# izhengfan/se2lam

Hardware: AMD Instinct MI355X
Metric: BA GN-iters/s (200 KF, 20k pts) (higher is better)
Workload: dtype f64; 1 GPU; globalBA-window 200 KF / 20000 landmarks / 119817 EdgeSE2XYZ + 199 PreEdgeSE2, LM optimize(10) (config 4 formulation, SURVEY D3); parallelism=single GPU

## Files before the change

se2lam_amd/csrc/ba.hip:

```cpp
#include <algorithm>
#include <atomic>
#include <chrono>
#include <cmath>
#include <cstdlib>
#include <functional>
#include <limits>
#include <mutex>
#include <thread>
#include <tuple>
#include <memory>
#include <unordered_map>

#include "common.h"
#include "se3_math.h"
#include "ba_device.h"
#include "ba_window.h"

using namespace se2gpu;
using namespace se2gpu::badev;

namespace {



// ... 154 lines not shown
        }
    }
}
template <bool FUSED>
__global__ __launch_bounds__(kBlock) void k_linearize(CamDev cam, int L, const int* __restrict__ lm_ptr,
                                                       const int* __restrict__ e_kf, const double* __restrict__ e_uv,
                                                       const double* __restrict__ e_info,
                                                       const double* __restrict__ poses,
                                                       const uint8_t* __restrict__ fixed,
                                                       const double* __restrict__ lms, double* W,
                                                       double* Hpp_e, double* bp_e,
                                                       double* __restrict__ Hll, double* __restrict__ bl, double lambda,
                                                       double* __restrict__ Ainv, double* __restrict__ zeta,
                                                       double* __restrict__ Dg,
                                                       const BaCtl* __restrict__ ctl, const double* __restrict__ poses_b,
                                                       const double* __restrict__ lms_b) {
    d_linearize<FUSED>(blockIdx.x, cam, L, lm_ptr, e_kf, e_uv, e_info, poses, fixed, lms, W, Hpp_e, bp_e, Hll, bl, lambda, Ainv, zeta, Dg, ctl, poses_b, lms_b);
}


__device__ __forceinline__ void d_odometry(const unsigned bx, int O, const int* __restrict__ o_i, const int* __restrict__ o_j,
                           const double* __restrict__ o_meas, const double* __restrict__ o_info,
                           const double* __restrict__ poses, const uint8_t* __restrict__ fixed,
                           double* __restrict__ Oii, double* __restrict__ Ojj, double* __restrict__ Oij,
                           double* __restrict__ obi, double* __restrict__ obj, const BaCtl* __restrict__ ctl,
                           const double* __restrict__ poses_b) {
    if (ctl && ctl->sel) poses = poses_b;
    const int k = bx * blockDim.x + threadIdx.x;
    if (k >= O) return;
    const int i = o_i[k], j = o_j[k];
    double e[3], A[9], B[9];
// ... 195 lines not shown
    const int i = o_i[k], j = o_j[k];
    pre_se2(poses + 3 * i, poses + 3 * j, o_meas + 3 * k, e, A, B);
    const double* W = o_info + 9 * k;
    for (int r = 0; r < 3; ++r) {
        omr[r] = -(W[r * 3] * e[0] + W[r * 3 + 1] * e[1] + W[r * 3 + 2] * e[2]);
        for (int c = 0; c < 3; ++c) {
            WA[r * 3 + c] = W[r * 3] * A[c] + W[r * 3 + 1] * A[3 + c] + W[r * 3 + 2] * A[6 + c];
            WB[r * 3 + c] = W[r * 3] * B[c] + W[r * 3 + 1] * B[3 + c] + W[r * 3 + 2] * B[6 + c];
        }
    }
}

constexpr int kGrpPerWG = 28;
constexpr int kChunk = 16;

__device__ __forceinline__ void d_reduce2(const unsigned bx, int P, int ld, int nwg_off, double lambda, int root,
                                                     const int4* __restrict__ grp, const int* __restrict__ blk_a,
                                                     const int* __restrict__ blk_b, const int* __restrict__ pair_i,
                                                     const int* __restrict__ pair_j, const int* __restrict__ blk_odo,
                                                     const double* __restrict__ W,
                                                     const double* __restrict__ Dg,
                                                     const uint8_t* __restrict__ fixed, const int* __restrict__ pose_ptr,
                                                     const int* __restrict__ pose_edges, const int* __restrict__ podo_ptr,
                                                     const int* __restrict__ podo_item, const int* __restrict__ o_i,
                                                     const int* __restrict__ o_j, const double* __restrict__ o_meas,
                                                     const double* __restrict__ o_info, const double* __restrict__ poses,
                                                     double* __restrict__ S, double* __restrict__ bp,
                                                     const BaCtl* __restrict__ ctl, const double* __restrict__ poses_b,
                                                     unsigned* __restrict__ epoch, const int* __restrict__ pose_off, int nsys) {
    const int n = pose_off ? nsys : 3 * P;
    __shared__ double part[kGrpPerWG][9];
    __shared__ double dpart[kBlock / 64][12];
    const int ndiag = (P + 1 + 7) & ~7;
    if ((int)bx >= ndiag) {
        const int bid = (int)bx - ndiag;
        const int nwg_pad = (nwg_off + 7) & ~7;
        const int wg = (bid & 7) * (nwg_pad >> 3) + (bid >> 3);
        if (wg >= nwg_off) return;
        const int lane = threadIdx.x & 63, gw = lane / 9, en = lane - 9 * gw;
        const int g = gw < 7 ? (int)(threadIdx.x >> 6) * 7 + gw : kGrpPerWG;
        int4 d = make_int4(-1, 0, 0, 0);
        if (g < kGrpPerWG) d = grp[(size_t)wg * kGrpPerWG + g];
        if (ctl) {
            if (ctl->done) return;
// ... 52 lines not shown
            for (int t = 0; t < ng; ++t) tot += part[g + t][en];
            double out = 0.0;
            if (free_ab) {
                out = -tot;
                if (od >= 0) {
                    double e[3], A[9], B[9], WA[9], WB[9], omr[3];
                    odo_terms(poses, fixed, o_i, o_j, o_meas, o_info, od >> 1, e, A, B, WA, WB, omr);
                    const int rr = (od & 1) ? c : r, cc = (od & 1) ? r : c;
                    const double a0 = rr == 0 ? A[0] : (rr == 1 ? A[1] : A[2]), a1 = rr == 0 ? A[3] : (rr == 1 ? A[4] : A[5]),
                                 a2 = rr == 0 ? A[6] : (rr == 1 ? A[7] : A[8]);
                    const double b0 = cc == 0 ? WB[0] : (cc == 1 ? WB[1] : WB[2]), b1 = cc == 0 ? WB[3] : (cc == 1 ? WB[4] : WB[5]),
                                 b2 = cc == 0 ? WB[6] : (cc == 1 ? WB[7] : WB[8]);
                    out += a0 * b0 + a1 * b1 + a2 * b2;
                }
            }
            S[(size_t)(ca + r) * ld + cb + c] = out;
            S[(size_t)(cb + c) * ld + ca + r] = out;
        }
        return;
    }
    if (ctl) {
        if (ctl->done) return;
        if (ctl->sel) poses = poses_b;
        lambda = ctl->lambda;
    }
    const int p = (int)bx;
    if (p > P) return;
    const int lane = threadIdx.x & 63, wv = threadIdx.x >> 6;
    double* __restrict__ bs = S + (size_t)n * ld;
    if (p == P) {
        for (size_t t = (size_t)n * ld + n + threadIdx.x; t < (size_t)ld * ld; t += kBlock) S[t] = 0.0;
        if (threadIdx.x == 0) {
            S[(size_t)ld * ld + 2] = 0.0;
            *epoch += 1u;
        }
        return;
    }
    double acc[12] = {0, 0, 0, 0, 0, 0, 0, 0, 0, 0, 0, 0};
    const bool fa = fixed[p];
    __shared__ double odoc[8][12];
    const int no = fa ? 0 : podo_ptr[p + 1] - podo_ptr[p];
    if ((int)threadIdx.x >= kBlock - 8 && (int)threadIdx.x - (kBlock - 8) < min(no, 8)) {
        const int t = podo_ptr[p] + (int)threadIdx.x - (kBlock - 8);
        const int k = podo_item[t] >> 1, isj = podo_item[t] & 1;
        double e[3], A[9], B[9], WA[9], WB[9], omr[3];
        odo_terms(poses, fixed, o_i, o_j, o_meas, o_info, k, e, A, B, WA, WB, omr);
        double J[9], WJ[9];
// ... 54 lines not shown
#pragma unroll
            for (int q = 0; q < 3; ++q) {
                const double j0 = isj ? B[3 * q] : A[3 * q], j1 = isj ? B[3 * q + 1] : A[3 * q + 1], j2 = isj ? B[3 * q + 2] : A[3 * q + 2];
                const double w0 = isj ? WB[3 * q] : WA[3 * q], w1 = isj ? WB[3 * q + 1] : WA[3 * q + 1], w2 = isj ? WB[3 * q + 2] : WA[3 * q + 2];
                jr[q] = r == 0 ? j0 : (r == 1 ? j1 : j2);
                wc[q] = i < 9 ? (c == 0 ? w0 : (c == 1 ? w1 : w2)) : omr[q];
            }
            v += jr[0] * wc[0] + jr[1] * wc[1] + jr[2] * wc[2];
        }
        if (i < 9) {
            const int r = i / 3, c = i - 3 * r;
            double out;
            if (fa) out = (r == c && root) ? 1.0 : 0.0;
            else out = v + ((r == c && root) ? lambda : 0.0);
            const int cp = pose_off ? pose_off[p] : 3 * p;
            S[(size_t)(cp + r) * ld + cp + c] = out;
        } else {
            const int r = i - 9;
            const double gz = dpart[0][9 + r] + dpart[1][9 + r] + dpart[2][9 + r] + dpart[3][9 + r];
            bs[(pose_off ? pose_off[p] : 3 * p) + r] = fa ? 0.0 : v - gz;
            bp[(size_t)p * 3 + r] = fa ? 0.0 : v;
        }
    }
}
__global__ __launch_bounds__(kBlock) void k_reduce2(int P, int ld, int nwg_off, double lambda, int root,
                                                     const int4* __restrict__ grp, const int* __restrict__ blk_a,
                                                     const int* __restrict__ blk_b, const int* __restrict__ pair_i,
                                                     const int* __restrict__ pair_j, const int* __restrict__ blk_odo,
                                                     const double* __restrict__ W,
                                                     const double* __restrict__ Dg,
                                                     const uint8_t* __restrict__ fixed, const int* __restrict__ pose_ptr,
                                                     const int* __restrict__ pose_edges, const int* __restrict__ podo_ptr,
                                                     const int* __restrict__ podo_item, const int* __restrict__ o_i,
                                                     const int* __restrict__ o_j, const double* __restrict__ o_meas,
                                                     const double* __restrict__ o_info, const double* __restrict__ poses,
                                                     double* __restrict__ S, double* __restrict__ bp,
                                                     const BaCtl* __restrict__ ctl, const double* __restrict__ poses_b,
                                                     unsigned* __restrict__ epoch, const int* __restrict__ pose_off, int nsys) {
// ... 212 lines not shown
        if (wall_clock64() - t0 > 200000000ll) return false;
    }
    return true;
}

constexpr int kVfyRecords = 64, kVfyChk = 8 + 8 * kVfyRecords;
__device__ inline unsigned long long wave_xor64(unsigned long long v) {
#pragma unroll
    for (int m = 1; m < 64; m <<= 1) v ^= (unsigned long long)__shfl_xor((long long)v, m);
    return v;
}
__device__ inline unsigned long long bits4(d2_t a, d2_t b) {
    return (unsigned long long)__double_as_longlong(a.x) ^ (unsigned long long)__double_as_longlong(a.y) ^
           (unsigned long long)__double_as_longlong(b.x) ^ (unsigned long long)__double_as_longlong(b.y);
}
template <bool VERIFY>
__device__ __forceinline__ void d_chol_tiles(const unsigned bx_dispatch, const double* __restrict__ A, double* __restrict__ PUB,
                                                     double* __restrict__ YU, int ld, int n,
                                                     int nbc, const int4* __restrict__ tasks, const int* __restrict__ deps,
                                                     const int* __restrict__ col_src,
                                                     unsigned* __restrict__ flagA, unsigned* __restrict__ flagR,
                                                     const unsigned* __restrict__ epoch_ptr, double* __restrict__ fail,
                                                     long long* __restrict__ dbg, const BaCtl* __restrict__ ctl,
                                                     double* __restrict__ xout, unsigned long long* __restrict__ vfy,
                                                     unsigned long long* __restrict__ head, int ntask) {
    if (ctl && ctl->done) return;
    __shared__ unsigned task_s;
    if (head) {
        if (threadIdx.x == 0) {
            const unsigned c = __hip_atomic_fetch_add(reinterpret_cast<unsigned*>(head), 1u, __ATOMIC_RELAXED, __HIP_MEMORY_SCOPE_AGENT);
            if (c == (unsigned)ntask - 1u) __hip_atomic_store(reinterpret_cast<unsigned*>(head), 0u, __ATOMIC_RELAXED, __HIP_MEMORY_SCOPE_AGENT);
// ... 61 lines not shown
        acc += __shfl_xor(acc, 4);
        if ((tid & 7) == 0 && kNB * r + row < n) {
            const int dst = col_src ? col_src[kNB * r + row] : kNB * r + row;
            if (dst >= 0) xout[dst] = acc;
        }
        return;
    }
    const bool isR = (tk.x >> 16) != 0;
    const int i = tk.x & 0xffff, j = tk.y;
    const bool isDiag = !isR && i == j;
    const int wv = tid >> 6, ln = tid & 63;
    const int qi = 16 * (wv >> 1), qj = 16 * (wv & 1);
    const int orow = qi + (ln >> 4), ocol = qj + (ln & 15);
    const int arow = ln & 15, acol = ln >> 4;
    d4_t T0 = {0, 0, 0, 0}, D0, accT = {0, 0, 0, 0}, accD = {0, 0, 0, 0};
#pragma unroll
    for (int v = 0; v < 4; ++v) {
        D0[v] = A[(size_t)(kNB * j + orow + 4 * v) * ld + kNB * j + ocol];
        if (!isR && !isDiag) T0[v] = A[(size_t)(kNB * i + orow + 4 * v) * ld + kNB * j + ocol];
    }
    const int sr = ln >> 1, sc = 8 * wv + 4 * (ln & 1);
    for (int dq = tk.z; dq < tk.w; ++dq) {
        const int dep = deps_s[dq - tk.z];
        const int m = dep & 0x7fff;
        const bool hasT = (dep >> 15) != 0;
        __syncthreads();
        if (!ok_s) {
            if (tid == 0) fail[0] = 1e6;
            return;
        }
        const bool lazy = dq + 1 < tk.w;
        const unsigned* f0 = flagA + ((size_t)j * nbc + m) * kSlabs + wv;
        const unsigned* f1 = hasT ? (isR ? flagR : flagA) + ((size_t)i * nbc + m) * kSlabs + wv : f0;
        const int need = dq - tk.z + 1;
// ... 205 lines not shown
    if (stamp && tid == 192) stamp[5] = wall_clock64();
}
template <bool VERIFY>
__global__ __launch_bounds__(256) void k_chol_tiles(const double* __restrict__ A, double* __restrict__ PUB,
                                                     double* __restrict__ YU, int ld, int n,
                                                     int nbc, const int4* __restrict__ tasks, const int* __restrict__ deps,
                                                     const int* __restrict__ col_src,
                                                     unsigned* __restrict__ flagA, unsigned* __restrict__ flagR,
                                                     const unsigned* __restrict__ epoch_ptr, double* __restrict__ fail,
                                                     long long* __restrict__ dbg, const BaCtl* __restrict__ ctl,
                                                     double* __restrict__ xout, unsigned long long* __restrict__ vfy,
                                                     unsigned long long* __restrict__ head, int ntask) {
    d_chol_tiles<VERIFY>(blockIdx.x, A, PUB, YU, ld, n, nbc, tasks, deps, col_src, flagA, flagR, epoch_ptr, fail, dbg, ctl, xout, vfy, head, ntask);
}

__global__ __launch_bounds__(256) void k_chol_apply(const double* __restrict__ A, const double* __restrict__ R, int ld,
                                                     int n, double* __restrict__ x, const BaCtl* __restrict__ ctl,
                                                     const int* __restrict__ col_src) {
    if (ctl && ctl->done) return;
    const int r = blockIdx.x * 4 + threadIdx.x / 64;
    const int lane = threadIdx.x & 63;
    if (r >= n) return;
    const double* y = A + (size_t)n * ld;
    double acc = 0.0;
    for (int c = r + lane; c < n; c += 64) acc += R[(size_t)r * ld + c] * y[c];
    acc = wave_sum(acc);
    const int dst = col_src ? col_src[r] : r;
    if (lane == 0 && dst >= 0) x[dst] = acc;
}

// ... 1353 lines not shown
    DevBuf<double> Hpl, Hpp_e, bp_e, Hll, bl, Dinv, z, Y, Dg, Hpp, bp, Oii, Ojj, Oij, obi, obj;
    DevBuf<double> red_own, xp, part, scal, diag3, Rinv;
    DevBuf<double> red_packed;
    DevBuf<int4> chol_tasks;
    DevBuf<int> chol_deps;
    DevBuf<int> pose_off;
    DevBuf<int> col_src;
    std::vector<int> h_pose_off;
    DevBuf<uint8_t> plan_nz;
    DevBuf<double> plan_nzd;
    PinBuf<uint8_t> h_plan_nz;
    DevBuf<uint8_t> solver_arena;
    int nsys = 0;
    int solve_depth = 0;
    DevBuf<unsigned> chol_flags;
    DevBuf<unsigned long long> chol_head;
    DevBuf<unsigned long long> chol_vfy;
    DevBuf<int> plan_place;
    DevBuf<unsigned> fin_counter;
    DevBuf<unsigned long long> l0_acc;
    int chol_ntask = 0;
    struct GraphSlot { int iters = -1, mode = -1; hipGraphExec_t exec = nullptr; unsigned long stamp = 0; };
    static constexpr int kGraphSlots = 3;
    GraphSlot graphs[kGraphSlots];
    unsigned long graph_clock = 0;
    void drop_graphs() {
        for (auto& g : graphs) {
            if (g.exec) (void)hipGraphExecDestroy(g.exec);
            g = GraphSlot{};
        }
// ... 725 lines not shown
        if (sw_best != w) ring(w, sw_best, 0);
    }
}

int ba_copy_stream(int device, hipStream_t* out) {
    static std::mutex mu;
    static hipStream_t streams[64] = {};
    std::lock_guard<std::mutex> lk(mu);
    SE2_REQUIRE(device >= 0 && device < 64, SE2GPU_ERR_INVALID, "device %d", device);
    if (!streams[device]) SE2_HIP(hipStreamCreateWithFlags(&streams[device], hipStreamNonBlocking));
    *out = streams[device];
    return SE2GPU_OK;
}

int ba_allreduce(se2gpu_ba* h, double* ptr, size_t count);

int ba_upload_graph(se2gpu_ba* h) {
    static const bool trace = [] { const char* e = getenv("SE2GPU_BA_INIT_TRACE"); return e && e[0] == '1'; }();
    const auto t_begin = std::chrono::steady_clock::now();
    auto lap = [&](const char* what) {
        if (trace)
            std::fprintf(stderr, "[ba init] %-28s %8.1f us\n", what,
                         std::chrono::duration<double, std::micro>(std::chrono::steady_clock::now() - t_begin).count());
    };
    const int P = (int)h->pose_ids.size(), L = (int)h->lm_ids.size();
    const int E = h->bulk_E ? h->bulk_E : (int)h->he_kf.size(), O_in = h->model ? (int)h->odo3.size() : (int)h->odo.size();
    const int D = h->D, ps = h->ps, gpw = h->model ? kGrpPerWG3 : kGrpPerWG;
    const int DS = D * (D + 1) / 2;
    SE2_REQUIRE(P > 0, SE2GPU_ERR_STATE, "initialize: no pose vertices");
    SE2_REQUIRE(!h->model || (h->world == 1 && !h->allreduce), SE2GPU_ERR_STATE, "the SE3 model is single-GPU");
// ... 482 lines not shown
        SE2_HIP(hipMemsetAsync(h->chol_flags.p, 0, 2 * kSlabs * (size_t)nt2 * nbc2 * sizeof(unsigned), st));
        SE2_CHECK(h->chol_head.reserve(1));
        SE2_HIP(hipMemsetAsync(h->chol_head.p, 0, sizeof(unsigned long long), st));
        static const bool verify = [] { const char* e = getenv("SE2GPU_BA_CHOL_VERIFY"); return e && e[0] == '1'; }();
        if (verify) {
            const size_t words = kVfyChk + 2 * 2 * kSlabs * (size_t)nt2 * nbc2;
            SE2_CHECK(h->chol_vfy.reserve(words));
            SE2_HIP(hipMemsetAsync(h->chol_vfy.p, 0, words * sizeof(unsigned long long), st));
        } else {
            h->chol_vfy.release();
        }
        const char* env = getenv("SE2GPU_BA_CHOL");
        h->chol_steps = (env && std::strcmp(env, "steps") == 0) || nt2 > 64 || h->chol_fallback;
        const char* tr = getenv("SE2GPU_BA_CHOL_TRACE");
        if (tr && tr[0] == '1') {
            SE2_CHECK(h->chol_trace.reserve(16 * (size_t)h->chol_ntask));
            SE2_HIP(hipMemsetAsync(h->chol_trace.p, 0, 16 * (size_t)h->chol_ntask * sizeof(long long), st));
        }
        lap("solve plan");
    }
    SE2_HIP(hipStreamSynchronize(st));
    if (device_plan) {
        int nwg = 0;
        std::memcpy(&nwg, h->h_scal.p, sizeof(int));
        SE2_REQUIRE(nwg <= h->grp_cap_wg, SE2GPU_ERR_CAPACITY, "device plan: %d workgroups exceed the bound %d", nwg, h->grp_cap_wg);
        h->nwg_off = std::max(nwg, 1);
    }
    lap("synchronise");
    h->bulk_E = 0;
    h->bulk_kf = h->bulk_lm = nullptr;
    h->bulk_uv = h->bulk_info = nullptr;
    h->initialized = true;
    h->est_valid = false;
    static std::atomic<unsigned long> serial{0};
    h->init_serial = ++serial;
    drain.armed = false;
    return SE2GPU_OK;
}


inline int ba_join(se2gpu_ba* h) {
    if (h->join_event) {
// ... 18 lines not shown
    const unsigned stride = gridDim.x * 256, t0 = blockIdx.x * 256 + threadIdx.x;
    for (unsigned i = t0; i < it.np; i += stride) it.dst_p[i] = it.src_p[i];
    for (unsigned i = t0; i < it.nl; i += stride) it.dst_l[i] = it.src_l[i];
}

struct Bufs {
    const BaCtl* c;
    double *pa, *pb, *la, *lb;
};
inline Bufs bufs(se2gpu_ba* h, bool ctl) {
    if (ctl) return Bufs{h->ctl.p, h->poses_a.p, h->poses_b.p, h->lms_a.p, h->lms_b.p};
    return Bufs{nullptr, h->poses, h->poses_t, h->lms, h->lms_t};
}


int ba_linearize(se2gpu_ba* h, double fuse_lambda, bool ctl = false) {
    hipStream_t st = h->stream;
    const Bufs B = bufs(h, ctl);
    if (h->model == 2) {
        SE2_LAUNCH(h->prof, st, "k4_terms", k4_terms, grid1((size_t)h->P + h->O, 64), dim3(64), 0, h->P, h->O, B.pa, h->fixed.p,
                   h->prior_has.p, h->prior_meas.p, h->prior_info.p, h->ph.p, h->pb.p, h->slot_a.p, h->slot_ptr.p, h->pe_i.p,
                   h->pe_j.p, h->pe_meas.p, h->pe_info.p, h->Oii.p, h->Ojj.p, h->Oij.p, h->obi.p, h->obj.p, B.c, B.pb);
        SE2_HIP(hipGetLastError());
        return SE2GPU_OK;
    }
    if (h->model) {
        if (fuse_lambda >= 0.0)
            SE2_LAUNCH(h->prof, st, "k3_linearize", (k3_linearize<true>), grid1((size_t)h->L * kGroup, kBlock), dim3(kBlock), 0,
                       h->cam3, h->L, h->lm_ptr.p, h->e_kf.p, h->e_uv.p, h->e_info.p, B.pa, h->fixed.p, B.la, h->Hpl.p,
                       h->Hpp_e.p, h->bp_e.p, h->Hll.p, h->bl.p, fuse_lambda, h->Dinv.p, h->z.p, h->Y.p, h->Dg.p, B.c, B.pb, B.lb);
        else
            SE2_LAUNCH(h->prof, st, "k3_linearize", (k3_linearize<false>), grid1((size_t)h->L * kGroup, kBlock), dim3(kBlock), 0,
                       h->cam3, h->L, h->lm_ptr.p, h->e_kf.p, h->e_uv.p, h->e_info.p, B.pa, h->fixed.p, B.la, h->Hpl.p,
                       h->Hpp_e.p, h->bp_e.p, h->Hll.p, h->bl.p, 0.0, h->Dinv.p, h->z.p, h->Y.p, h->Dg.p, B.c, B.pb, B.lb);
        SE2_LAUNCH(h->prof, st, "k3_terms", k3_terms, grid1((size_t)h->P + h->O, 64), dim3(64), 0, h->P, h->O, B.pa, h->fixed.p,
                   h->prior_has.p, h->prior_meas.p, h->prior_info.p, h->pb.p, h->o_i.p, h->o_j.p, h->o_meas.p, h->o_info.p,
                   h->Oii.p, h->Ojj.p, h->Oij.p, h->obi.p, h->obj.p, B.c, B.pb);
        SE2_HIP(hipGetLastError());
        return SE2GPU_OK;
    }
    if (fuse_lambda >= 0.0)
        SE2_LAUNCH(h->prof, st, "k_linearize", (k_linearize<true>), grid1((size_t)h->L * kGroup, kBlock), dim3(kBlock), 0,
                   h->cam, h->L, h->lm_ptr.p, h->e_kf.p, h->e_uv.p, h->e_info.p, B.pa, h->fixed.p, B.la, h->Hpl.p,
                   h->Hpp_e.p, h->bp_e.p, h->Hll.p, h->bl.p, fuse_lambda, h->Dinv.p, h->z.p, h->Dg.p, B.c, B.pb, B.lb);
    else
        SE2_LAUNCH(h->prof, st, "k_linearize0", (k_linearize<false>), grid1((size_t)h->L * kGroup, kBlock), dim3(kBlock), 0,
                   h->cam, h->L, h->lm_ptr.p, h->e_kf.p, h->e_uv.p, h->e_info.p, B.pa, h->fixed.p, B.la, h->Hpl.p,
                   h->Hpp_e.p, h->bp_e.p, h->Hll.p, h->bl.p, 0.0, h->Dinv.p, h->z.p, h->Dg.p, B.c, B.pb, B.lb);
    SE2_HIP(hipGetLastError());
    return SE2GPU_OK;
}

int ba_pose_blocks(se2gpu_ba* h, const double* poses, bool ctl = false, bool odometry_only = false) {
    hipStream_t st = h->stream;
    if (h->O) {
        if (ctl)
            SE2_LAUNCH(h->prof, st, "k_odometry", k_odometry, grid1(h->O, 64), dim3(64), 0, h->O, h->o_i.p, h->o_j.p,
                       h->o_meas.p, h->o_info.p, h->poses_a.p, h->fixed.p, h->Oii.p, h->Ojj.p, h->Oij.p, h->obi.p, h->obj.p,
                       (const BaCtl*)h->ctl.p, (const double*)h->poses_b.p);
        else
            SE2_LAUNCH(h->prof, st, "k_odometry", k_odometry, grid1(h->O, 64), dim3(64), 0, h->O, h->o_i.p, h->o_j.p,
                       h->o_meas.p, h->o_info.p, poses, h->fixed.p, h->Oii.p, h->Ojj.p, h->Oij.p, h->obi.p, h->obj.p,
                       (const BaCtl*)nullptr, (const double*)nullptr);
    }
    if (!odometry_only)
        SE2_LAUNCH(h->prof, st, "k_pose_reduce", k_pose_reduce, grid1((size_t)h->P * 64, kBlock), dim3(kBlock), 0, h->P,
                   h->pose_ptr.p, h->pose_edges.p, h->Hpp_e.p, h->bp_e.p, h->podo_ptr.p, h->podo_item.p, h->Oii.p,
                   h->Ojj.p, h->obi.p, h->obj.p, h->Hpp.p, h->bp.p);
    SE2_HIP(hipGetLastError());
    return SE2GPU_OK;
}

int ba_reduce(se2gpu_ba* h, double lambda, int schur, bool ctl = false) {
    hipStream_t st = h->stream;
    double* S = h->red;
    const Bufs B = bufs(h, ctl);
    if (h->model) {
        const double* pinfo = h->model == 2 ? h->ph.p : h->prior_info.p;
        if (schur && h->model == 1)
            SE2_LAUNCH(h->prof, st, "k3_schur_lm", k3_schur_lm, grid1((size_t)h->L * kGroup, kBlock), dim3(kBlock), 0, h->L,
                       lambda, h->lm_ptr.p, h->Hll.p, h->bl.p, h->Hpl.p, h->Hpp_e.p, h->bp_e.p, h->Dinv.p, h->z.p, h->Y.p,
                       h->Dg.p, B.c, schur == 2 ? 0 : 1);
        SE2_LAUNCH(h->prof, st, "k3_reduce2", k3_reduce2, dim3(((h->P + 1 + 7) & ~7) + ((h->nwg_off + 7) & ~7)), dim3(kBlock), 0,
                   h->P, h->ld, h->nwg_off, lambda, h->grp.p, h->blk_a.p, h->blk_b.p, h->pair_i.p, h->pair_j.p, h->blk_odo.p,
                   h->Y.p, h->Hpl.p, h->Dg.p, h->fixed.p, h->pose_ptr.p, h->pose_edges.p, h->podo_ptr.p, h->podo_item.p,
                   h->prior_has.p, pinfo, h->pb.p, h->Oii.p, h->Ojj.p, h->Oij.p, h->obi.p, h->obj.p, S, h->bp.p, B.c,
                   &h->ctl.p->epoch);
        SE2_HIP(hipGetLastError());
        return SE2GPU_OK;
    }
    if (schur) SE2_CHECK(ba_linearize(h, lambda, ctl));
    SE2_LAUNCH(h->prof, st, "k_reduce2", k_reduce2, dim3(((h->P + 1 + 7) & ~7) + ((h->nwg_off + 7) & ~7)), dim3(kBlock), 0, h->P, h->ld, h->nwg_off,
               lambda, h->root, h->grp.p, h->blk_a.p, h->blk_b.p, h->pair_i.p, h->pair_j.p, h->blk_odo.p,
               h->Hpl.p, h->Dg.p, h->fixed.p, h->pose_ptr.p, h->pose_edges.p,
               h->podo_ptr.p, h->podo_item.p, h->o_i.p, h->o_j.p, h->o_meas.p, h->o_info.p, B.pa, S, h->bp.p, B.c, B.pb,
               &h->ctl.p->epoch, (const int*)h->pose_off.p, h->nsys);
    if (h->O && h->odo_fallback) {
        SE2_LAUNCH(h->prof, st, "k_odometry", k_odometry, grid1(h->O, 64), dim3(64), 0, h->O, h->o_i.p, h->o_j.p,
                   h->o_meas.p, h->o_info.p, h->poses, h->fixed.p, h->Oii.p, h->Ojj.p, h->Oij.p, h->obi.p, h->obj.p,
                   (const BaCtl*)nullptr, (const double*)nullptr);
        SE2_LAUNCH(h->prof, st, "k_reduce_odo", k_reduce_odo, grid1((size_t)h->O * 9, 256), dim3(256), 0, h->O, h->ld,
                   h->o_i.p, h->o_j.p, h->Oij.p, S);
    }
    SE2_HIP(hipGetLastError());
    return SE2GPU_OK;
}
// ... 145 lines not shown
        const int skip = (fault && !h->chol_faulted && h->chol_ntask > 1) ? 1 : 0;
        h->chol_faulted = true;
        if (h->chol_vfy.p)
            SE2_LAUNCH(h->prof, st, "k_chol_tiles", k_chol_tiles<true>, dim3(h->chol_ntask - skip), dim3(256), 0, A, Rm, YU, ld, n, nbc,
                       h->chol_tasks.p + skip, (const int*)h->chol_deps.p, (const int*)h->col_src.p, flagA, flagR, &h->ctl.p->epoch,
                       fail, h->chol_trace.p, c, h->xp.p, h->chol_vfy.p, head, h->chol_ntask - skip);
        else
            SE2_LAUNCH(h->prof, st, "k_chol_tiles", k_chol_tiles<false>, dim3(h->chol_ntask - skip), dim3(256), 0, A, Rm, YU, ld, n, nbc,
                       h->chol_tasks.p + skip, (const int*)h->chol_deps.p, (const int*)h->col_src.p, flagA, flagR, &h->ctl.p->epoch,
                       fail, h->chol_trace.p, c, h->xp.p, (unsigned long long*)nullptr, head, h->chol_ntask - skip);
    }
    SE2_HIP(hipGetLastError());
    return SE2GPU_OK;
}

int ba_lambda_init(se2gpu_ba* h) {
    hipStream_t st = h->stream;
    if (h->model) {
        SE2_LAUNCH(h->prof, st, "k3_pose_diag", k3_pose_diag, grid1((size_t)h->P * 64, kBlock), dim3(kBlock), 0, h->P,
                   h->pose_ptr.p, h->pose_edges.p, h->Hpp_e.p, h->fixed.p, h->prior_has.p,
                   h->model == 2 ? h->ph.p : h->prior_info.p, h->podo_ptr.p, h->podo_item.p, h->Oii.p, h->Ojj.p, h->diag3.p);
        SE2_LAUNCH(h->prof, st, "k_maxdiag", k_maxdiag, dim3(1), dim3(1024), 0, h->L, h->Hll.p, h->P, h->diag3.p,
                   h->fixed.p, h->scal.p, 6, 0, h->ctl.p);
        SE2_HIP(hipGetLastError());
        return SE2GPU_OK;
    }
    const bool sharded = h->allreduce && h->world > 1;
    const size_t nd = 3 * (size_t)h->P;
    if (!sharded) {
        SE2_CHECK(ba_pose_blocks(h, h->poses, true, true));
// ... 71 lines not shown
                   0.0, h->lm_ptr.p, h->e_kf.p, h->e_uv.p, h->e_info.p, B.pa, h->fixed.p, B.la,
                   step ? h->xp.p : (const double*)nullptr, h->z.p, (const double*)h->Hpl.p, h->bl.p, B.lb, h->part.p, B.c, B.pb, FinArgs{},
                   (const double*)h->Dinv.p);
        SE2_LAUNCH(h->prof, st, "k_finalize", k_finalize, dim3(1), dim3(1024), 0, h->L ? h->nparts : 0, h->part.p, h->P,
                   0.0, B.pa, h->fixed.p, h->xp.p, h->bp.p, B.pb, h->O, h->o_i.p, h->o_j.p, h->o_meas.p,
                   h->o_info.p, h->root, scal, h->d_mail, seq, h->ctl.p, step ? 1 : 0, sharded ? 0 : 1, note ? 1 : 0,
                   (const volatile int*)h->d_stop);
        if (sharded) {
            SE2_CHECK(ba_allreduce(h, scal, 4));
            hipLaunchKernelGGL(k_lm_decide, dim3(1), dim3(256), 0, st, h->ctl.p, scal, step ? 1 : 0, note ? 1 : 0,
                               h->d_mail, seq, (const volatile int*)h->d_stop);
        }
        SE2_HIP(hipGetLastError());
        return SE2GPU_OK;
    };
    if (first) {
        SE2_CHECK(evaluate(false, false));
        if (lm) {
            SE2_CHECK(ba_linearize(h, -1.0, true));
            SE2_CHECK(ba_lambda_init(h));
            SE2_CHECK(ba_reduce(h, 0.0, 3, true));
        } else {
            SE2_CHECK(ba_linearize(h, 0.0, true));
            SE2_CHECK(ba_reduce(h, 0.0, 0, true));
        }
    } else {
        if (know_retry != 1) SE2_CHECK(ba_linearize(h, 0.0, true));
        SE2_CHECK(ba_reduce(h, 0.0, !lm ? 0 : know_retry == 0 ? 0 : know_retry == 1 ? 3 : (h->model ? 2 : 0), true));
    }
    SE2_CHECK(ba_allreduce_system(h));
    SE2_CHECK(ba_solve(h, true));
    SE2_CHECK(evaluate(true, notify));
    return SE2GPU_OK;
}


template <typename... A>
struct Packed {
    int nblk;
    std::tuple<A...> args;
};
template <auto Body, int BS, typename... A>
__global__ __launch_bounds__(BS) void k_batched(const Packed<A...>* __restrict__ p) {
// ... 1613 lines not shown
```

Measured before the change: 6519 iters/s.

## Fuse Schur reduction into tiled Cholesky kernel with per-tile readiness counters

Merges the reduced-camera-system assembly (k_reduce2) into the dataflow Cholesky launch. Reduction blocks publish S entries with agent-scope stores and bump per-32x32-tile ready counters. Cholesky task blocks spin until the tiles they need are complete, using an expected-count table precomputed at setup and scaled by a generation counter bumped in linearize. This removes a kernel boundary so factorization can overlap assembly, at the cost of spin-waits, atomics on every S write, and a co-residency requirement checked through occupancy.

```diff
diff --git a/se2lam_amd/csrc/ba.hip b/se2lam_amd/csrc/ba.hip
--- a/se2lam_amd/csrc/ba.hip
+++ b/se2lam_amd/csrc/ba.hip
@@ -192,7 +192,13 @@
                                                        double* __restrict__ Ainv, double* __restrict__ zeta,
                                                        double* __restrict__ Dg,
                                                        const BaCtl* __restrict__ ctl, const double* __restrict__ poses_b,
-                                                       const double* __restrict__ lms_b) {
+                                                       const double* __restrict__ lms_b, unsigned* __restrict__ prep_epoch,
+                                                       unsigned long long* __restrict__ prep_gen, double* __restrict__ prep_fail) {
+    if (prep_gen && blockIdx.x == 0 && threadIdx.x == 0 && !(ctl && ctl->done)) {
+        *prep_epoch += 1u;
+        *prep_gen += 1ull;
+        *prep_fail = 0.0;
+    }
     d_linearize<FUSED>(blockIdx.x, cam, L, lm_ptr, e_kf, e_uv, e_info, poses, fixed, lms, W, Hpp_e, bp_e, Hll, bl, lambda, Ainv, zeta, Dg, ctl, poses_b, lms_b);
 }
 
@@ -418,7 +424,20 @@
 constexpr int kGrpPerWG = 28;
 constexpr int kChunk = 16;
 
-__device__ __forceinline__ void d_reduce2(const unsigned bx, int P, int ld, int nwg_off, double lambda, int root,
+constexpr int kSTile = 32;
+template <bool PUB>
+__device__ __forceinline__ void s_put(double* __restrict__ S, int ld, int row, int col, double v, unsigned* tl, int nt) {
+    double* p = S + (size_t)row * ld + col;
+    if constexpr (PUB) {
+        __hip_atomic_store(p, v, __ATOMIC_RELAXED, __HIP_MEMORY_SCOPE_AGENT);
+        const int ti = row / kSTile, tj = col / kSTile;
+        if (ti >= tj) atomicOr(tl + ((ti * nt + tj) >> 5), 1u << ((ti * nt + tj) & 31));
+    } else {
+        *p = v;
+    }
+}
+template <bool PUB>
+__device__ __forceinline__ void d_reduce2_body(const unsigned bx, int P, int ld, int nwg_off, double lambda, int root,
                                                      const int4* __restrict__ grp, const int* __restrict__ blk_a,
                                                      const int* __restrict__ blk_b, const int* __restrict__ pair_i,
                                                      const int* __restrict__ pair_j, const int* __restrict__ blk_odo,
@@ -431,7 +450,8 @@
                                                      const double* __restrict__ o_info, const double* __restrict__ poses,
                                                      double* __restrict__ S, double* __restrict__ bp,
                                                      const BaCtl* __restrict__ ctl, const double* __restrict__ poses_b,
-                                                     unsigned* __restrict__ epoch, const int* __restrict__ pose_off, int nsys) {
+                                                     unsigned* __restrict__ epoch, const int* __restrict__ pose_off, int nsys,
+                                                     unsigned* tl = nullptr, int nt = 0) {
     const int n = pose_off ? nsys : 3 * P;
     __shared__ double part[kGrpPerWG][9];
     __shared__ double dpart[kBlock / 64][12];
@@ -514,8 +534,8 @@
                     out += a0 * b0 + a1 * b1 + a2 * b2;
                 }
             }
-            S[(size_t)(ca + r) * ld + cb + c] = out;
-            S[(size_t)(cb + c) * ld + ca + r] = out;
+            s_put<PUB>(S, ld, ca + r, cb + c, out, tl, nt);
+            s_put<PUB>(S, ld, cb + c, ca + r, out, tl, nt);
         }
         return;
     }
@@ -527,10 +547,9 @@
     const int p = (int)bx;
     if (p > P) return;
     const int lane = threadIdx.x & 63, wv = threadIdx.x >> 6;
-    double* __restrict__ bs = S + (size_t)n * ld;
     if (p == P) {
-        for (size_t t = (size_t)n * ld + n + threadIdx.x; t < (size_t)ld * ld; t += kBlock) S[t] = 0.0;
-        if (threadIdx.x == 0) {
+        for (size_t t = (size_t)n * ld + n + threadIdx.x; t < (size_t)ld * ld; t += kBlock) s_put<PUB>(S, ld, (int)(t / ld), (int)(t % ld), 0.0, tl, nt);
+        if (threadIdx.x == 0 && epoch) {
             S[(size_t)ld * ld + 2] = 0.0;
             *epoch += 1u;
         }
@@ -615,14 +634,30 @@
             if (fa) out = (r == c && root) ? 1.0 : 0.0;
             else out = v + ((r == c && root) ? lambda : 0.0);
             const int cp = pose_off ? pose_off[p] : 3 * p;
-            S[(size_t)(cp + r) * ld + cp + c] = out;
+            s_put<PUB>(S, ld, cp + r, cp + c, out, tl, nt);
         } else {
             const int r = i - 9;
             const double gz = dpart[0][9 + r] + dpart[1][9 + r] + dpart[2][9 + r] + dpart[3][9 + r];
-            bs[(pose_off ? pose_off[p] : 3 * p) + r] = fa ? 0.0 : v - gz;
+            s_put<PUB>(S, ld, n, (pose_off ? pose_off[p] : 3 * p) + r, fa ? 0.0 : v - gz, tl, nt);
             bp[(size_t)p * 3 + r] = fa ? 0.0 : v;
         }
     }
+}
+__device__ __forceinline__ void d_reduce2(const unsigned bx, int P, int ld, int nwg_off, double lambda, int root,
+                                          const int4* __restrict__ grp, const int* __restrict__ blk_a,
+                                          const int* __restrict__ blk_b, const int* __restrict__ pair_i,
+                                          const int* __restrict__ pair_j, const int* __restrict__ blk_odo,
+                                          const double* __restrict__ W, const double* __restrict__ Dg,
+                                          const uint8_t* __restrict__ fixed, const int* __restrict__ pose_ptr,
+                                          const int* __restrict__ pose_edges, const int* __restrict__ podo_ptr,
+                                          const int* __restrict__ podo_item, const int* __restrict__ o_i,
+                                          const int* __restrict__ o_j, const double* __restrict__ o_meas,
+                                          const double* __restrict__ o_info, const double* __restrict__ poses,
+                                          double* __restrict__ S, double* __restrict__ bp,
+                                          const BaCtl* __restrict__ ctl, const double* __restrict__ poses_b,
+                                          unsigned* __restrict__ epoch, const int* __restrict__ pose_off, int nsys) {
+    d_reduce2_body<false>(bx, P, ld, nwg_off, lambda, root, grp, blk_a, blk_b, pair_i, pair_j, blk_odo, W, Dg, fixed, pose_ptr, pose_edges,
+                          podo_ptr, podo_item, o_i, o_j, o_meas, o_info, poses, S, bp, ctl, poses_b, epoch, pose_off, nsys);
 }
 __global__ __launch_bounds__(kBlock) void k_reduce2(int P, int ld, int nwg_off, double lambda, int root,
                                                      const int4* __restrict__ grp, const int* __restrict__ blk_a,
@@ -865,7 +900,7 @@
     return (unsigned long long)__double_as_longlong(a.x) ^ (unsigned long long)__double_as_longlong(a.y) ^
            (unsigned long long)__double_as_longlong(b.x) ^ (unsigned long long)__double_as_longlong(b.y);
 }
-template <bool VERIFY>
+template <bool VERIFY, bool SAGENT = false>
 __device__ __forceinline__ void d_chol_tiles(const unsigned bx_dispatch, const double* __restrict__ A, double* __restrict__ PUB,
                                                      double* __restrict__ YU, int ld, int n,
                                                      int nbc, const int4* __restrict__ tasks, const int* __restrict__ deps,
@@ -957,10 +992,26 @@
     const int orow = qi + (ln >> 4), ocol = qj + (ln & 15);
     const int arow = ln & 15, acol = ln >> 4;
     d4_t T0 = {0, 0, 0, 0}, D0, accT = {0, 0, 0, 0}, accD = {0, 0, 0, 0};
-#pragma unroll
-    for (int v = 0; v < 4; ++v) {
-        D0[v] = A[(size_t)(kNB * j + orow + 4 * v) * ld + kNB * j + ocol];
-        if (!isR && !isDiag) T0[v] = A[(size_t)(kNB * i + orow + 4 * v) * ld + kNB * j + ocol];
+    if constexpr (SAGENT) {
+        d2_t q[4], z0 = {0, 0}, z1 = {0, 0};
+#pragma unroll
+        for (int v = 0; v < 4; ++v) q[v] = load_agent(A + (size_t)(kNB * j + orow + 4 * v) * ld + kNB * j + (ocol & ~1));
+        SE2_WAIT_VM6(q[0], q[1], q[2], q[3], z0, z1);
+#pragma unroll
+        for (int v = 0; v < 4; ++v) D0[v] = (ocol & 1) ? q[v].y : q[v].x;
+        if (!isR && !isDiag) {
+#pragma unroll
+            for (int v = 0; v < 4; ++v) q[v] = load_agent(A + (size_t)(kNB * i + orow + 4 * v) * ld + kNB * j + (ocol & ~1));
+            SE2_WAIT_VM6(q[0], q[1], q[2], q[3], z0, z1);
+#pragma unroll
+            for (int v = 0; v < 4; ++v) T0[v] = (ocol & 1) ? q[v].y : q[v].x;
+        }
+    } else {
+#pragma unroll
+        for (int v = 0; v < 4; ++v) {
+            D0[v] = A[(size_t)(kNB * j + orow + 4 * v) * ld + kNB * j + ocol];
+            if (!isR && !isDiag) T0[v] = A[(size_t)(kNB * i + orow + 4 * v) * ld + kNB * j + ocol];
+        }
     }
     const int sr = ln >> 1, sc = 8 * wv + 4 * (ln & 1);
     for (int dq = tk.z; dq < tk.w; ++dq) {
@@ -1196,6 +1247,106 @@
     d_chol_tiles<VERIFY>(blockIdx.x, A, PUB, YU, ld, n, nbc, tasks, deps, col_src, flagA, flagR, epoch_ptr, fail, dbg, ctl, xout, vfy, head, ntask);
 }
 
+struct Reduce2Args {
+    int P, ld, nwg_off;
+    double lambda;
+    int root;
+    const int4* grp;
+    const int *blk_a, *blk_b, *pair_i, *pair_j, *blk_odo;
+    const double *W, *Dg;
+    const uint8_t* fixed;
+    const int *pose_ptr, *pose_edges, *podo_ptr, *podo_item, *o_i, *o_j;
+    const double *o_meas, *o_info, *poses;
+    double *S, *bp;
+    const BaCtl* ctl;
+    const double* poses_b;
+    const int* pose_off;
+    int nsys;
+};
+static_assert(kNB == kSTile, "the tile-ready counters count tiles of the dense solve");
+constexpr int kTileWords = 64 * 64 / 32;
+
+__device__ __forceinline__ void d_reduce_task(unsigned bx, const Reduce2Args& a, int nt, unsigned long long* __restrict__ ready) {
+    __shared__ unsigned tl[kTileWords];
+    for (int t = threadIdx.x; t < kTileWords; t += kBlock) tl[t] = 0u;
+    __syncthreads();
+    d_reduce2_body<true>(bx, a.P, a.ld, a.nwg_off, a.lambda, a.root, a.grp, a.blk_a, a.blk_b, a.pair_i, a.pair_j, a.blk_odo, a.W, a.Dg,
+                         a.fixed, a.pose_ptr, a.pose_edges, a.podo_ptr, a.podo_item, a.o_i, a.o_j, a.o_meas, a.o_info, a.poses, a.S, a.bp,
+                         a.ctl, a.poses_b, (unsigned*)nullptr, a.pose_off, a.nsys, tl, nt);
+    asm volatile("s_waitcnt vmcnt(0)" ::: "memory");
+    __syncthreads();
+    const int words = (nt * nt + 31) >> 5;
+    for (int w = threadIdx.x; w < words; w += kBlock) {
+        unsigned m = tl[w];
+        while (m) {
+            const int b = __builtin_ctz(m);
+            m &= m - 1u;
+            __hip_atomic_fetch_add(ready + 32 * w + b, 1ull, __ATOMIC_RELAXED, __HIP_MEMORY_SCOPE_AGENT);
+        }
+    }
+}
+__global__ __launch_bounds__(kBlock) void k_chol_fused_expect(Reduce2Args a, unsigned long long* __restrict__ expect) {
+    d_reduce_task(blockIdx.x, a, a.ld / kNB, expect);
+}
+__device__ inline bool ready_wait(const unsigned long long* c, unsigned long long want) {
+    const long long t0 = wall_clock64();
+    while (__hip_atomic_load(c, __ATOMIC_RELAXED, __HIP_MEMORY_SCOPE_AGENT) != want) {
+        __builtin_amdgcn_s_sleep(2);
+        if (wall_clock64() - t0 > 200000000ll) return false;
+    }
+    return true;
+}
+template <bool VERIFY>
+__global__ __launch_bounds__(256) void k_chol_tiles_fused(Reduce2Args ra, int nred, unsigned long long* __restrict__ ready,
+                                                          const unsigned long long* __restrict__ expect,
+                                                          const unsigned long long* __restrict__ gen_ptr,
+                                                          const double* __restrict__ A, double* __restrict__ PUB,
+                                                          double* __restrict__ YU, int ld, int n,
+                                                          int nbc, const int4* __restrict__ tasks, const int* __restrict__ deps,
+                                                          const int* __restrict__ col_src,
+                                                          unsigned* __restrict__ flagA, unsigned* __restrict__ flagR,
+                                                          const unsigned* __restrict__ epoch_ptr, double* __restrict__ fail,
+                                                          long long* __restrict__ dbg, const BaCtl* __restrict__ ctl,
+                                                          double* __restrict__ xout, unsigned long long* __restrict__ vfy,
+                                                          unsigned long long* __restrict__ head, int ntask) {
+    if (ctl && ctl->done) return;
+    const int nt = ld / kNB;
+    if ((int)blockIdx.x < nred) {
+        if (dbg && blockIdx.x == 0 && threadIdx.x == 0) dbg[16 * (size_t)ntask] = wall_clock64();
+        d_reduce_task(blockIdx.x, ra, nt, ready);
+        return;
+    }
+    __shared__ unsigned task_s;
+    __shared__ int ok_s;
+    if (threadIdx.x == 0) {
+        const unsigned c = __hip_atomic_fetch_add(reinterpret_cast<unsigned*>(head), 1u, __ATOMIC_RELAXED, __HIP_MEMORY_SCOPE_AGENT);
+        if (c == (unsigned)ntask - 1u) __hip_atomic_store(reinterpret_cast<unsigned*>(head), 0u, __ATOMIC_RELAXED, __HIP_MEMORY_SCOPE_AGENT);
+        task_s = c;
+        ok_s = 1;
+    }
+    __syncthreads();
+    const unsigned t = task_s;
+    const int4 tk = tasks[t];
+    if ((tk.x >> 16) != 2) {
+        if (threadIdx.x == 0) {
+            long long* stamp = dbg ? dbg + (size_t)t * 16 : nullptr;
+            if (stamp) stamp[8] = wall_clock64();
+            const unsigned long long g = *gen_ptr;
+            const int i = tk.x & 0xffff, j = tk.y;
+            const int td = j * nt + j, tt = ((tk.x >> 16) == 0 && i != j) ? i * nt + j : td;
+            ok_s = (ready_wait(ready + td, expect[td] * g) && ready_wait(ready + tt, expect[tt] * g)) ? 1 : 0;
+            if (stamp) stamp[9] = wall_clock64();
+        }
+        __syncthreads();
+        if (!ok_s) {
+            if (threadIdx.x == 0) fail[0] = 1e6;
+            return;
+        }
+    }
+    d_chol_tiles<VERIFY, true>(t, A, PUB, YU, ld, n, nbc, tasks, deps, col_src, flagA, flagR, epoch_ptr, fail, dbg, ctl, xout, vfy,
+                               (unsigned long long*)nullptr, ntask);
+}
+
 __global__ __launch_bounds__(256) void k_chol_apply(const double* __restrict__ A, const double* __restrict__ R, int ld,
                                                      int n, double* __restrict__ x, const BaCtl* __restrict__ ctl,
                                                      const int* __restrict__ col_src) {
@@ -2579,6 +2730,8 @@
     int nsys = 0;
     int solve_depth = 0;
     DevBuf<unsigned> chol_flags;
+    DevBuf<unsigned long long> fz;
+    bool fused = false;
     DevBuf<unsigned long long> chol_head;
     DevBuf<unsigned long long> chol_vfy;
     DevBuf<int> plan_place;
@@ -3334,6 +3487,38 @@
 }
 
 int ba_allreduce(se2gpu_ba* h, double* ptr, size_t count);
+
+Reduce2Args ba_reduce2_args(se2gpu_ba* h, const BaCtl* ctl, const double* poses, const double* poses_b) {
+    return Reduce2Args{h->P, h->ld, h->nwg_off, 0.0, h->root, h->grp.p, h->blk_a.p, h->blk_b.p, h->pair_i.p, h->pair_j.p,
+                       h->blk_odo.p, h->Hpl.p, h->Dg.p, h->fixed.p, h->pose_ptr.p, h->pose_edges.p, h->podo_ptr.p, h->podo_item.p,
+                       h->o_i.p, h->o_j.p, h->o_meas.p, h->o_info.p, poses, h->red, h->bp.p, ctl, poses_b,
+                       (const int*)h->pose_off.p, h->nsys};
+}
+inline int ba_reduce2_grid(const se2gpu_ba* h) { return ((h->P + 1 + 7) & ~7) + ((h->nwg_off + 7) & ~7); }
+
+bool ba_fused_solve_ok(const se2gpu_ba* h) {
+    static const bool on = [] { const char* e = getenv("SE2GPU_BA_FUSED_SOLVE"); return !(e && e[0] == '0'); }();
+    static const int capacity = [] {
+        int per_cu = 0, dev = 0;
+        hipDeviceProp_t pr{};
+        if (hipGetDevice(&dev) != hipSuccess || hipGetDeviceProperties(&pr, dev) != hipSuccess) return 0;
+        if (hipOccupancyMaxActiveBlocksPerMultiprocessor(&per_cu, reinterpret_cast<const void*>(&k_chol_tiles_fused<false>), 256, 0) != hipSuccess) return 0;
+        return per_cu * pr.multiProcessorCount;
+    }();
+    return on && h->model == 0 && !h->allreduce && !h->ar_buffer && !h->odo_fallback && !h->host_solve && !h->chol_steps &&
+           h->ld / kNB <= 64 && h->chol_ntask > 0 && 2 * h->chol_ntask <= capacity;
+}
+int ba_fused_setup(se2gpu_ba* h) {
+    h->fused = ba_fused_solve_ok(h);
+    if (!h->fused) return SE2GPU_OK;
+    const size_t nt = (size_t)h->ld / kNB, words = 1 + 2 * nt * nt;
+    SE2_CHECK(h->fz.reserve(words));
+    SE2_HIP(hipMemsetAsync(h->fz.p, 0, words * sizeof(unsigned long long), h->stream));
+    hipLaunchKernelGGL(k_chol_fused_expect, dim3(ba_reduce2_grid(h)), dim3(kBlock), 0, h->stream,
+                       ba_reduce2_args(h, (const BaCtl*)nullptr, h->poses, h->poses), h->fz.p + 1 + nt * nt);
+    SE2_HIP(hipGetLastError());
+    return SE2GPU_OK;
+}
 
 int ba_upload_graph(se2gpu_ba* h) {
     static const bool trace = [] { const char* e = getenv("SE2GPU_BA_INIT_TRACE"); return e && e[0] == '1'; }();
@@ -3846,8 +4031,8 @@
         h->chol_steps = (env && std::strcmp(env, "steps") == 0) || nt2 > 64 || h->chol_fallback;
         const char* tr = getenv("SE2GPU_BA_CHOL_TRACE");
         if (tr && tr[0] == '1') {
-            SE2_CHECK(h->chol_trace.reserve(16 * (size_t)h->chol_ntask));
-            SE2_HIP(hipMemsetAsync(h->chol_trace.p, 0, 16 * (size_t)h->chol_ntask * sizeof(long long), st));
+            SE2_CHECK(h->chol_trace.reserve(16 * ((size_t)h->chol_ntask + 1)));
+            SE2_HIP(hipMemsetAsync(h->chol_trace.p, 0, 16 * ((size_t)h->chol_ntask + 1) * sizeof(long long), st));
         }
         lap("solve plan");
     }
@@ -3858,6 +4043,7 @@
         SE2_REQUIRE(nwg <= h->grp_cap_wg, SE2GPU_ERR_CAPACITY, "device plan: %d workgroups exceed the bound %d", nwg, h->grp_cap_wg);
         h->nwg_off = std::max(nwg, 1);
     }
+    SE2_CHECK(ba_fused_setup(h));
     lap("synchronise");
     h->bulk_E = 0;
     h->bulk_kf = h->bulk_lm = nullptr;
@@ -3906,7 +4092,7 @@
 }
 
 
-int ba_linearize(se2gpu_ba* h, double fuse_lambda, bool ctl = false) {
+int ba_linearize(se2gpu_ba* h, double fuse_lambda, bool ctl = false, bool prep = false) {
     hipStream_t st = h->stream;
     const Bufs B = bufs(h, ctl);
     if (h->model == 2) {
@@ -3934,11 +4120,14 @@
     if (fuse_lambda >= 0.0)
         SE2_LAUNCH(h->prof, st, "k_linearize", (k_linearize<true>), grid1((size_t)h->L * kGroup, kBlock), dim3(kBlock), 0,
                    h->cam, h->L, h->lm_ptr.p, h->e_kf.p, h->e_uv.p, h->e_info.p, B.pa, h->fixed.p, B.la, h->Hpl.p,
-                   h->Hpp_e.p, h->bp_e.p, h->Hll.p, h->bl.p, fuse_lambda, h->Dinv.p, h->z.p, h->Dg.p, B.c, B.pb, B.lb);
+                   h->Hpp_e.p, h->bp_e.p, h->Hll.p, h->bl.p, fuse_lambda, h->Dinv.p, h->z.p, h->Dg.p, B.c, B.pb, B.lb,
+                   prep ? &h->ctl.p->epoch : (unsigned*)nullptr, prep ? h->fz.p : (unsigned long long*)nullptr,
+                   prep ? h->red + (size_t)h->ld * h->ld + 2 : (double*)nullptr);
     else
         SE2_LAUNCH(h->prof, st, "k_linearize0", (k_linearize<false>), grid1((size_t)h->L * kGroup, kBlock), dim3(kBlock), 0,
                    h->cam, h->L, h->lm_ptr.p, h->e_kf.p, h->e_uv.p, h->e_info.p, B.pa, h->fixed.p, B.la, h->Hpl.p,
-                   h->Hpp_e.p, h->bp_e.p, h->Hll.p, h->bl.p, 0.0, h->Dinv.p, h->z.p, h->Dg.p, B.c, B.pb, B.lb);
+                   h->Hpp_e.p, h->bp_e.p, h->Hll.p, h->bl.p, 0.0, h->Dinv.p, h->z.p, h->Dg.p, B.c, B.pb, B.lb,
+                   (unsigned*)nullptr, (unsigned long long*)nullptr, (double*)nullptr);
     SE2_HIP(hipGetLastError());
     return SE2GPU_OK;
 }
@@ -3963,7 +4152,7 @@
     return SE2GPU_OK;
 }
 
-int ba_reduce(se2gpu_ba* h, double lambda, int schur, bool ctl = false) {
+int ba_reduce(se2gpu_ba* h, double lambda, int schur, bool ctl = false, bool fused = false) {
     hipStream_t st = h->stream;
     double* S = h->red;
     const Bufs B = bufs(h, ctl);
@@ -3981,7 +4170,8 @@
         SE2_HIP(hipGetLastError());
         return SE2GPU_OK;
     }
-    if (schur) SE2_CHECK(ba_linearize(h, lambda, ctl));
+    if (schur) SE2_CHECK(ba_linearize(h, lambda, ctl, fused));
+    if (fused) return SE2GPU_OK;
     SE2_LAUNCH(h->prof, st, "k_reduce2", k_reduce2, dim3(((h->P + 1 + 7) & ~7) + ((h->nwg_off + 7) & ~7)), dim3(kBlock), 0, h->P, h->ld, h->nwg_off,
                lambda, h->root, h->grp.p, h->blk_a.p, h->blk_b.p, h->pair_i.p, h->pair_j.p, h->blk_odo.p,
                h->Hpl.p, h->Dg.p, h->fixed.p, h->pose_ptr.p, h->pose_edges.p,
@@ -4157,6 +4347,39 @@
     return SE2GPU_OK;
 }
 
+int ba_solve_fused(se2gpu_ba* h) {
+    hipStream_t st = h->stream;
+    const int n = h->nsys, ld = h->ld;
+    const int nt = ld / kNB, nbc = (n + kNB - 1) / kNB;
+    double* A = h->red;
+    double* fail = h->red + (size_t)ld * ld + 2;
+    double* Rm = h->Rinv.p;
+    double* YU = Rm + 2 * (size_t)nt * nbc * kSlabs * kSlabDoubles;
+    unsigned* flagA = h->chol_flags.p;
+    unsigned* flagR = flagA + kSlabs * (size_t)nt * nbc;
+    const Bufs B = bufs(h, true);
+    const Reduce2Args ra = ba_reduce2_args(h, B.c, B.pa, B.pb);
+    const int nred = ba_reduce2_grid(h);
+    unsigned long long* ready = h->fz.p + 1;
+    const unsigned long long* expect = h->fz.p + 1 + (size_t)nt * nt;
+    static const bool fault = [] { const char* e = getenv("SE2GPU_BA_CHOL_FAULT"); return e && e[0] == '1'; }();
+    const int skip = (fault && !h->chol_faulted && h->chol_ntask > 1) ? 1 : 0;
+    h->chol_faulted = true;
+    const int ns = h->chol_ntask - skip;
+    if (h->chol_vfy.p)
+        SE2_LAUNCH(h->prof, st, "k_chol_tiles_fused", k_chol_tiles_fused<true>, dim3(nred + ns), dim3(256), 0, ra, nred, ready, expect,
+                   (const unsigned long long*)h->fz.p, A, Rm, YU, ld, n, nbc, h->chol_tasks.p + skip, (const int*)h->chol_deps.p,
+                   (const int*)h->col_src.p, flagA, flagR, &h->ctl.p->epoch, fail, h->chol_trace.p, B.c, h->xp.p, h->chol_vfy.p,
+                   h->chol_head.p, ns);
+    else
+        SE2_LAUNCH(h->prof, st, "k_chol_tiles_fused", k_chol_tiles_fused<false>, dim3(nred + ns), dim3(256), 0, ra, nred, ready, expect,
+                   (const unsigned long long*)h->fz.p, A, Rm, YU, ld, n, nbc, h->chol_tasks.p + skip, (const int*)h->chol_deps.p,
+                   (const int*)h->col_src.p, flagA, flagR, &h->ctl.p->epoch, fail, h->chol_trace.p, B.c, h->xp.p,
+                   (unsigned long long*)nullptr, h->chol_head.p, ns);
+    SE2_HIP(hipGetLastError());
+    return SE2GPU_OK;
+}
+
 int ba_lambda_init(se2gpu_ba* h) {
     hipStream_t st = h->stream;
     if (h->model) {
@@ -4258,19 +4481,26 @@
         SE2_HIP(hipGetLastError());
         return SE2GPU_OK;
     };
+    const bool fused = h->fused && !h->chol_steps && !sharded;
     if (first) {
         SE2_CHECK(evaluate(false, false));
         if (lm) {
             SE2_CHECK(ba_linearize(h, -1.0, true));
             SE2_CHECK(ba_lambda_init(h));
-            SE2_CHECK(ba_reduce(h, 0.0, 3, true));
+            SE2_CHECK(ba_reduce(h, 0.0, 3, true, fused));
         } else {
-            SE2_CHECK(ba_linearize(h, 0.0, true));
-            SE2_CHECK(ba_reduce(h, 0.0, 0, true));
+            SE2_CHECK(ba_linearize(h, 0.0, true, fused));
+            SE2_CHECK(ba_reduce(h, 0.0, 0, true, fused));
         }
     } else {
-        if (know_retry != 1) SE2_CHECK(ba_linearize(h, 0.0, true));
-        SE2_CHECK(ba_reduce(h, 0.0, !lm ? 0 : know_retry == 0 ? 0 : know_retry == 1 ? 3 : (h->model ? 2 : 0), true));
+        const int schur = !lm ? 0 : know_retry == 0 ? 0 : know_retry == 1 ? 3 : (h->model ? 2 : 0);
+        if (know_retry != 1) SE2_CHECK(ba_linearize(h, 0.0, true, fused && !schur));
+        SE2_CHECK(ba_reduce(h, 0.0, schur, true, fused));
+    }
+    if (fused) {
+        SE2_CHECK(ba_solve_fused(h));
+        SE2_CHECK(evaluate(true, notify));
+        return SE2GPU_OK;
     }
     SE2_CHECK(ba_allreduce_system(h));
     SE2_CHECK(ba_solve(h, true));
```

Result: slower. 6381 iters/s (median of 2 runs) (-2.1%).
